# mlpc-ucsd/BDM

Measured on AMD Instinct MI355X. Metric: sampled shapes/sec (4096 pts, 1000 DDPM steps), higher is better.
Workload: dtype f32

## Files before the change

bdm_amd/csrc/sparse_conv_os.hip:

```cpp
#include <stdlib.h>

#include "../../include/bdm_hip.h"
#include "common.h"

using namespace bdm;

#include "sparse_h2_common.h"

#define OS_PAIRS 14

typedef __attribute__((ext_vector_type(4))) float f32x4a;
typedef float f32x4v_t __attribute__((ext_vector_type(4)));


#define TILE_REC 16
#define DILH_XCAP 1376

static void sconv_dil_geometry(int r, int half_tile, int *tile, int *xcap, int *tiles_max) {
  if (half_tile > 0) {
    *tile = half_tile;
    *xcap = DILH_XCAP;
  } else {
    *tile = r == 32 ? 512 : (r == 16 ? 256 : 128);
    *xcap = 3 * r * r;
// ... 222 lines not shown

extern "C" int bdm_voxel_dilate_slices(int r, int tile) {
  int tl, xcap, tiles_max;
  sconv_dil_geometry(r, half_tile_ok(r, tile) ? tile : 0, &tl, &xcap, &tiles_max);
  return tiles_max;
}

static int voxel_dilate_launch(int b, int r, int n_dil_max, const int *src, int thr, int *dil_list, int *dil_index, int *plane_start,
                               int *tile_start, int *class_count, int half_tile, void *stream) {
  BDM_REQUIRE(b >= 0 && (r == 8 || r == 16 || r == 32) && n_dil_max >= 1 && src && dil_list && dil_index && plane_start && tile_start,
              "voxel_dilate: bad arguments (r in {8, 16, 32})");
  BDM_REQUIRE(half_tile_ok(r, half_tile), "voxel_dilate: tile %d unsupported (0 = full tiles; 64 / 128 / 256: EXPERIMENTAL=1 builds)", half_tile);
  if (b == 0) return BDM_OK;
  int tile, xcap, tiles_max;
  sconv_dil_geometry(r, half_tile, &tile, &xcap, &tiles_max);
  BDM_REQUIRE(cdiv(r * r * r, tile) <= 1024, "voxel_dilate: more flat tiles than threads");
  const size_t smem = sizeof(unsigned) * (4 * (size_t)r * r + 1 + 32 + 2 * (r + 2));
  hipLaunchKernelGGL(vox_dilate_kernel, dim3(b), dim3(1024), smem, (hipStream_t)stream, r, n_dil_max, tile, xcap, tiles_max,
                     half_tile > 0 ? 1 : 0, src, thr, dil_list, dil_index, plane_start, tile_start, class_count);
  return launch_status("voxel_dilate");
}

extern "C" int bdm_voxel_dilate(int b, int r, int n_dil_max, const int *cnt, int *dil_list, int *dil_index, int *plane_start,
                                int *tile_start, int tile, void *stream) {
  return voxel_dilate_launch(b, r, n_dil_max, cnt, 0, dil_list, dil_index, plane_start, tile_start, nullptr, tile, stream);
}

extern "C" int bdm_voxel_dilate_again(int b, int r, int n_dil_max, const int *dil_index_in, int *dil_list, int *dil_index,
                                      int *plane_start, int *tile_start, int *class_count, int tile, void *stream) {
  BDM_REQUIRE(class_count != nullptr, "voxel_dilate_again: class_count is NULL");
  return voxel_dilate_launch(b, r, n_dil_max, dil_index_in, -1, dil_list, dil_index, plane_start, tile_start, class_count, tile, stream);
}

#ifdef DIL_TIMING
__device__ long long *g_dil_ts = nullptr;
extern "C" int bdm_debug_dil_timestamps(long long *buf) { return hipMemcpyToSymbol(HIP_SYMBOL(g_dil_ts), &buf, sizeof(buf)) == hipSuccess ? 0 : 1; }
#define DIL_STAMP(i) do { if (g_dil_ts && tid == 0) { g_dil_ts[(size_t)item * 8 + (i)] = wall_clock64();                                  \
    if ((i) == 0) g_dil_ts[(size_t)item * 8 + 7] = (long long)__builtin_amdgcn_s_getreg(63492) | ((long long)__builtin_amdgcn_s_getreg(63508) << 32); } } while (0)
#else
#define DIL_STAMP(i)
#endif

template <int MT, int NT, int NW, int R, bool H2IN>
__global__ __launch_bounds__(NW * 64) void sconv_dil_kernel(
    int C8, int Cout, int n_max, int n_dil_max, int xcap, const float4 *__restrict__ xr, const float *__restrict__ amax,
    const float4 *__restrict__ xconst, float x_inv_scale,
    const int *__restrict__ occ_index, const int *__restrict__ dil_list, const int *__restrict__ dil_index,
    const int *__restrict__ tile_start, const float4 *__restrict__ wq,
    const float *__restrict__ inv_scale, const float *__restrict__ bias, float *__restrict__ y, int compact, int gn_cg,
    double *__restrict__ gn_partial, int gn_slices, int nb_shapes, int ncb, int tiles_max, int *__restrict__ work_counter) {
  extern __shared__ __align__(16) float4 smem4[];
  constexpr int BM = 16 * MT, TILE = NT * NW * 16;
  constexpr int R2 = R * R, R3 = R2 * R;
  constexpr int NT_ = NW * 64;
  constexpr int WV = OS_PAIRS * 2 * 2 * BM, WI = (WV + NT_ - 1) / NT_;
  constexpr int NQ = OS_PAIRS / 2;
  constexpr int PF = MT * NT >= 16 ? 1 : 2;
  constexpr int NBLK = NT * NW, NB = MT * 4 * 2;
  float4 *Ws = smem4;
  float4 *Xs = smem4 + WV;
  const int XS = xcap + 128;
  __shared__ int s_item;
  __shared__ float s_osc[64], s_obi[64];

  const int tid0 = threadIdx.x;
  const int G = gn_partial != nullptr ? Cout / gn_cg : 0, S = gn_slices;
  const int items = tiles_max * ncb * nb_shapes;
  for (;;) {
    int tid = tid0;
    asm volatile("" : "+v"(tid));
    const int lane = tid & 63, wave = tid >> 6, l16 = lane & 15, kg = lane >> 4;
    __syncthreads();
    if (tid == 0) s_item = atomicAdd(work_counter, 1);
    __syncthreads();
    const int item = s_item;
    if (item >= items) break;
    const int bi = item % nb_shapes, m0 = ((item / nb_shapes) % ncb) * BM, tile = item / (nb_shapes * ncb);
  const int4 *te = reinterpret_cast<const int4 *>(tile_start + ((size_t)bi * tiles_max + tile) * TILE_REC);
  const int4 ta = te[0], tb = te[1];
  const int j0 = ta.x, jn = ta.y, v_first = ta.z, v_end = ta.w, k_lo = tb.x;
  const int tiles_live = tb.w, tile_x0 = tb.z >> 8, tile_x1 = tb.z & 255;
// ... 62 lines not shown
      *reinterpret_cast<f16x8 *>(&Xs[row]) = hi;
      *reinterpret_cast<f16x8 *>(&Xs[XS + row]) = lo;
    }
  };
  auto store_chunk = [&](int c8) {
#pragma unroll
    for (int u = 0; u < PF; ++u)
      if (tid + u * NT_ < nrows) {
        const float4 p = make_float4(xa[u][0][0], xa[u][0][1], xa[u][0][2], xa[u][0][3]);
        const float4 q = make_float4(xa[u][1][0], xa[u][1][1], xa[u][1][2], xa[u][1][3]);
        put(tid + u * NT_, p, q);
      }
    for (int row0 = tid + PF * NT_; row0 < nrows; row0 += 2 * NT_) {
      const int row1 = row0 + NT_, rc1 = min(row1, nrows - 1);
      float4 a0, a1, b0, b1;
      if (H2IN) {
        const float4 *src = xr + (((size_t)bi * C8 + c8) * 2) * n_max + k_lo;
        a0 = src[row0]; a1 = src[n_max + row0]; b0 = src[rc1]; b1 = src[n_max + rc1];
      } else {
        const float4 *src = xb + ((size_t)c8 * n_max + k_lo) * 2;
        a0 = src[2 * row0]; a1 = src[2 * row0 + 1]; b0 = src[2 * rc1]; b1 = src[2 * rc1 + 1];
      }
      put(row0, a0, a1);
      if (row1 < nrows) put(row1, b0, b1);
    }
    if (H2IN && tid < 128) *reinterpret_cast<f32x4v *>(&Xs[(tid >> 6) * XS + xcap + 64 + (tid & 63)]) = cr;
#pragma unroll
    for (int i = 0; i < WI; ++i) {
      const int e = tid + i * NT_;
      if (e < WV) *reinterpret_cast<f32x4v *>(&Ws[e]) = wr[i];
    }
  };

  if (!nothing) load_chunk(0);

  int rec[NT][NQ];
  unsigned amask = 0u;
  {
    const int pl0 = max(tile_x0 - 1, 0), pl1 = min(tile_x1 + 1, R - 1), n_oi = (pl1 - pl0 + 1) * R2;
    const bool staged = !nothing && n_oi * (int)sizeof(int) <= 2 * XS * (int)sizeof(float4);
    int *s_oi = reinterpret_cast<int *>(Xs);
    const int *oi = occ_index + (size_t)bi * R3;
    int vq[NT];
#pragma unroll
    for (int q = 0; q < NT; ++q) {
      const int j = j0 + (q * NW + wave) * 16 + l16;
      vq[q] = j < jn ? dl[j] : -1;
    }
    if (staged) {
      const int4 *src = reinterpret_cast<const int4 *>(oi + pl0 * R2);
      for (int e = tid; e < n_oi / 4; e += NT_) reinterpret_cast<int4 *>(s_oi)[e] = src[e];
      __syncthreads();
    }
#pragma unroll
    for (int q = 0; q < NT; ++q) {
      const int v = vq[q];
      const int vx = v / R2, vy = (v / R) % R, vz = v % R;
#pragma unroll
      for (int Q = 0; Q < NQ; ++Q) {
        const int t = 4 * Q + kg;
        int k = -1;
        bool inside = false;
        if (v >= 0 && t < 27) {
          const int gx = vx + t / 9 - 1, gy = vy + (t / 3) % 3 - 1, gz = vz + t % 3 - 1;
          inside = gx >= 0 && gx < R && gy >= 0 && gy < R && gz >= 0 && gz < R;
          if (inside) k = staged ? s_oi[((gx - pl0) * R + gy) * R + gz] : oi[(gx * R + gy) * R + gz];
        }
        const bool here = k >= k_lo && k - k_lo < nrows;
        const bool live = here || (H2IN && inside);
        if (__ballot(live) != 0ull) amask |= 1u << (Q * NT + q);
        rec[q][Q] = here ? k - k_lo : ((H2IN && inside) ? xcap + 64 + lane : xcap + lane);
      }
    }
    amask = __builtin_amdgcn_readfirstlane(amask);
  }
  DIL_STAMP(1);
  if (!nothing) {
    for (int c8 = 0; c8 < C8; ++c8) {
      __syncthreads();
      if (c8 == 0) DIL_STAMP(2);
      if (c8 == 0 && tid < 128) Xs[(tid >> 6) * XS + xcap + (tid & 63)] = make_float4(0.f, 0.f, 0.f, 0.f);
      store_chunk(c8);
      __syncthreads();
      if (c8 == 0) DIL_STAMP(3);
      if (c8 == 1) DIL_STAMP(4);
      if (c8 + 1 < C8) load_chunk(c8 + 1);
#pragma unroll
      for (int Q = 0; Q < NQ; ++Q) {
        const unsigned qm = (amask >> (Q * NT)) & ((1u << NT) - 1u);
        if (qm == 0u) continue;
        f16x8 fa[MT][2];
#pragma unroll
        for (int s = 0; s < 2; ++s)
#pragma unroll
          for (int mt = 0; mt < MT; ++mt) {
            const float4 t = wbase[Q * 8 * BM + s * 2 * BM + mt * 16];
            fa[mt][s] = *reinterpret_cast<const f16x8 *>(&t);
          }
#pragma unroll
        for (int q = 0; q < NT; ++q) {
          f16x8 fb[2];
#pragma unroll
          for (int s = 0; s < 2; ++s) {
            const float4 t = Xs[s * XS + rec[q][Q]];
            fb[s] = *reinterpret_cast<const f16x8 *>(&t);
          }
#pragma unroll
          for (int term = 0; term < 3; ++term)
#pragma unroll
            for (int mt = 0; mt < MT; ++mt)
              acc[mt][q] = __builtin_amdgcn_mfma_f32_16x16x32_f16(fa[mt][term == 0 ? 1 : 0], fb[term == 1 ? 1 : 0], acc[mt][q], 0, 0, 0);
        }
      }
    }
  }

  DIL_STAMP(5);
  __syncthreads();
  float *red = reinterpret_cast<float *>(smem4);
  float *otile = red + (NBLK + 1) * NB;
#pragma unroll
  for (int mt = 0; mt < MT; ++mt)
#pragma unroll
    for (int q = 0; q < NT; ++q) {
      const int jl = (q * NW + wave) * 16 + l16;
      const bool live = j0 + jl < jn;
      float bs = 0.f, bq = 0.f;
      f32x4a o = f32x4a{0.f, 0.f, 0.f, 0.f};
#pragma unroll
      for (int i = 0; i < 4; ++i) {
        const int m = m0 + mt * 16 + 4 * kg + i;
        if (m < Cout && live) {
          const float v = acc[mt][q][i] * s_osc[mt * 16 + 4 * kg + i] + s_obi[mt * 16 + 4 * kg + i];
          o[i] = v;
          bs += v;
          bq = __builtin_fmaf(v, v, bq);
        }
// ... 368 lines not shown
        float a = 0.f;
#pragma unroll
        for (int j = 0; j < NBLK; ++j) a += red[j * NB + e];
        red2[e] = a;
      }
      __syncthreads();
      const int ngt = BM / gn_cg;
      if (tid < ngt && m0 + tid * gn_cg < Cout) {
        double a = 0.0, qq = 0.0;
        const int nb4 = gn_cg / 4;
        for (int j = 0; j < nb4; ++j) {
          a += (double)red2[(tid * nb4 + j) * 2 + 0];
          qq += (double)red2[(tid * nb4 + j) * 2 + 1];
        }
        const double nfill = H2IN ? 0.0 : (double)((v_end - v_first) - (jn - j0));
        for (int c = 0; c < gn_cg; ++c) {
          const double bv = bias ? (double)bias[m0 + tid * gn_cg + c] : 0.0;
          a += nfill * bv;
          qq += nfill * bv * bv;
        }
        double *dst = gn_partial + (((size_t)bi * G + m0 / gn_cg + tid) * S + tile) * 2;
        dst[0] = a;
        dst[1] = qq;
      }
    }
    DIL_STAMP(6);
  }
}

#endif

static int sconv_dil_launch(bool h2in, int b, int cin, int cout, int r, int n_max, int n_dil_max, const void *xr, const float *amax,
                            const void *xconst, float x_inv_scale, const int *in_index, const int *dil_list, const int *dil_index,
                            const int *tile_start, const void *packed_w, const float *inv_scale, const float *bias, float *y,
                            int compact, int gn_cg, double *gn_partial, int *slices_out, int half_tile, int *work_counter,
                            void *stream) {
  BDM_REQUIRE(b >= 0 && cin >= 1 && cout >= 1 && n_max >= 1 && n_dil_max >= 1 && xr && (h2in ? xconst != nullptr : amax != nullptr) &&
                  in_index && dil_list && dil_index && tile_start && inv_scale && y && work_counter,
              "sparse_conv_dil: bad arguments");
  if (r != 8 && r != 16 && r != 32) {
    set_error("sparse_conv_dil: resolution %d unsupported (8, 16, 32)", r);
    return BDM_ERR_UNSUPPORTED;
  }
  BDM_REQUIRE(half_tile_ok(r, half_tile), "sparse_conv_dil: tile %d unsupported (0 = full tiles; 64 / 128 / 256: EXPERIMENTAL=1 builds)", half_tile);
  if (b == 0) return BDM_OK;
  const int c8 = (cin + 7) / 8;
  const int mi = cout > 32 ? 2 : 1;
  int tile, xcap, tiles;
  sconv_dil_geometry(r, half_tile, &tile, &xcap, &tiles);
  const int bm = 32 * mi, nblk = tile / 16, nb = (bm / 16) * 8, ncb = cdiv(cout, bm);
  size_t smem = half_tile ? 16 * (2 * ((size_t)xcap + 128))
                          : 16 * ((size_t)OS_PAIRS * 4 * bm + 2 * ((size_t)xcap + 128));
  const size_t smem_out = sizeof(float) * ((size_t)(nblk + 1) * nb + (compact ? 0 : (size_t)bm * tile));
  if (smem_out > smem) smem = smem_out;
  BDM_REQUIRE(!half_tile || smem + 1024 <= 81920, "sparse_conv_dil: the half-tile form needs two workgroups per CU (%zu bytes of LDS)", smem);
  static int cus[16] = {0};
  int dev = 0;
  (void)hipGetDevice(&dev);
  if (dev < 0 || dev >= 16 || cus[dev] == 0) {
    hipDeviceProp_t prop;
    const int n = hipGetDeviceProperties(&prop, dev) == hipSuccess ? prop.multiProcessorCount : 256;
    if (dev >= 0 && dev < 16) cus[dev] = n > 0 ? n : 256;
  }
  const int ncu = ((dev >= 0 && dev < 16) ? cus[dev] : 256) * (half_tile ? 2 : 1);
  const long long items = (long long)tiles * ncb * b;
  dim3 grid((unsigned)(items < ncu ? items : ncu));
  hipStream_t s = (hipStream_t)stream;
  const int slices = h2in ? tiles + 27 : tiles;
  if (gn_partial != nullptr) {
    BDM_REQUIRE(gn_cg >= 4 && (gn_cg & (gn_cg - 1)) == 0 && bm % gn_cg == 0 && cout % gn_cg == 0,
                "sparse_conv_dil: GroupNorm statistics need a power-of-two channels-per-group dividing %d (got cg=%d)", bm, gn_cg);
    if (slices_out) *slices_out = slices;
  }
#define DIL_LAUNCH_(MT, NT, NW, R, H)                                                                                      \
  do {                                                                                                                     \
    BDM_ALLOW_LDS((sconv_dil_kernel<MT, NT, NW, R, H>), smem);                                                             \
    hipLaunchKernelGGL((sconv_dil_kernel<MT, NT, NW, R, H>), grid, dim3(NW * 64), smem, s, c8, cout, n_max, n_dil_max,     \
                       xcap, (const float4 *)xr, amax, (const float4 *)xconst, x_inv_scale, in_index, dil_list, dil_index, \
                       tile_start, (const float4 *)packed_w, inv_scale, bias, y, compact, gn_cg, gn_partial, slices, b,    \
                       ncb, tiles, work_counter);                                                                          \
  } while (0)
#define DIL_LAUNCH(MT, NT, NW, R) do { if (h2in) DIL_LAUNCH_(MT, NT, NW, R, true); else DIL_LAUNCH_(MT, NT, NW, R, false); } while (0)
#define DILH_LAUNCH_(MT, NT, R, H)                                                                                         \
  do {                                                                                                                     \
    BDM_ALLOW_LDS((sconv_dilh_kernel<MT, NT, R, H>), smem);                                                                \
    hipLaunchKernelGGL((sconv_dilh_kernel<MT, NT, R, H>), grid, dim3(256), smem, s, c8, cout, n_max, n_dil_max,            \
                       (const float4 *)xr, amax, (const float4 *)xconst, x_inv_scale, in_index, dil_list, dil_index,       \
                       tile_start, (const float4 *)packed_w, inv_scale, bias, y, compact, gn_cg, gn_partial, slices, b,    \
                       ncb, tiles, work_counter);                                                                          \
  } while (0)
#define DILH_LAUNCH(MT, NT, R) do { if (h2in) DILH_LAUNCH_(MT, NT, R, true); else DILH_LAUNCH_(MT, NT, R, false); } while (0)
#define DILH_PICK(NT, R) do { if (mi == 2) DILH_LAUNCH(4, NT, R); else DILH_LAUNCH(2, NT, R); } while (0)
#ifdef BDM_EXPERIMENTAL
  if (half_tile) {
    const int nt = half_tile / 64;
    if (r == 32) { if (nt == 4) DILH_PICK(4, 32); else if (nt == 2) DILH_PICK(2, 32); else DILH_PICK(1, 32); }
    else if (r == 16) { if (nt == 4) DILH_PICK(4, 16); else if (nt == 2) DILH_PICK(2, 16); else DILH_PICK(1, 16); }
    else { if (nt == 2) DILH_PICK(2, 8); else DILH_PICK(1, 8); }
    return launch_status("sparse_conv_dil (half tiles)");
  }
#endif
  if (r == 32) { if (mi == 2) DIL_LAUNCH(4, 4, 8, 32); else DIL_LAUNCH(2, 4, 8, 32); }
  else if (r == 16) { if (mi == 2) DIL_LAUNCH(4, 2, 8, 16); else DIL_LAUNCH(2, 2, 8, 16); }
  else { if (mi == 2) DIL_LAUNCH(4, 1, 8, 8); else DIL_LAUNCH(2, 1, 8, 8); }
#undef DIL_LAUNCH
#undef DIL_LAUNCH_
#undef DILH_PICK
#undef DILH_LAUNCH
#undef DILH_LAUNCH_
  return launch_status("sparse_conv_dil");
}

extern "C" int bdm_sparse_conv_dil(int b, int cin, int cout, int r, int n_max, int n_dil_max, const void *xr, const float *amax,
                                   const int *occ_index, const int *dil_list, const int *dil_index, const int *tile_start,
                                   const void *packed_w, const float *inv_scale, const float *bias, float *y,
                                   int compact, int tile, int *work_counter, void *stream) {
  return sconv_dil_launch(false, b, cin, cout, r, n_max, n_dil_max, xr, amax, nullptr, 0.f, occ_index, dil_list, dil_index, tile_start,
                          packed_w, inv_scale, bias, y, compact, 0, nullptr, nullptr, tile, work_counter, stream);
}

extern "C" int bdm_sparse_conv_dil_gn(int b, int cin, int cout, int r, int n_max, int n_dil_max, const void *xr, const float *amax,
                                      const int *occ_index, const int *dil_list, const int *dil_index, const int *tile_start,
                                      const void *packed_w, const float *inv_scale, const float *bias,
                                      float *y, int compact, int groups, void *gn_partial, int *slices_out, int tile,
                                      int *work_counter, void *stream) {
  BDM_REQUIRE(groups >= 1 && cout % groups == 0 && gn_partial != nullptr && slices_out != nullptr, "sparse_conv_dil_gn: bad arguments");
  return sconv_dil_launch(false, b, cin, cout, r, n_max, n_dil_max, xr, amax, nullptr, 0.f, occ_index, dil_list, dil_index, tile_start,
                          packed_w, inv_scale, bias, y, compact, cout / groups, (double *)gn_partial, slices_out, tile, work_counter, stream);
}

extern "C" int bdm_sparse_conv_dil_h2_gn(int b, int cin, int cout, int r, int n_rows_max, int n_dil_max, const void *rows_h2,
                                         const void *xconst, float x_inv_scale, const int *in_index, const int *dil_list,
                                         const int *dil_index, const int *tile_start, const void *packed_w, const float *inv_scale,
                                         const float *bias, float *y, int groups, void *gn_partial, int *slices_out, int tile,
                                         int *work_counter, void *stream) {
  BDM_REQUIRE(groups >= 1 && cout % groups == 0 && gn_partial != nullptr && slices_out != nullptr && x_inv_scale > 0.f,
              "sparse_conv_dil_h2_gn: bad arguments");
  return sconv_dil_launch(true, b, cin, cout, r, n_rows_max, n_dil_max, rows_h2, nullptr, xconst, x_inv_scale, in_index, dil_list,
                          dil_index, tile_start, packed_w, inv_scale, bias, y, 1, cout / groups, (double *)gn_partial, slices_out, tile,
                          work_counter, stream);
}
```

bdm_amd/ops.py:

```python
import ctypes
import os

import torch

from . import _lib as L
from . import tape


def _bcl(t):
    if t.dtype != torch.float32:
        raise L.BdmHipError(f"expected float32, got {t.dtype}")
    B, C = t.shape[0], t.shape[1]
    if B * C > 0 and t.is_contiguous():
        l = t.numel() // (B * C)
        return t, B, C, l, C * l, l
    l = 1
    for s in t.shape[2:]:
        l *= s
    dense, exp = True, 1
    for d in range(t.dim() - 1, 1, -1):
        if t.shape[d] != 1 and t.stride(d) != exp:
            dense = False
        exp *= t.shape[d]
    if dense and C > 1 and t.stride(1) < l:
# ... 794 lines not shown
_amax_rings = {}
_static_epoch = 0
_static_epochs = 0


class static_step:

    def __enter__(self):
        global _static_epoch, _static_epochs
        _static_epochs += 1
        _static_epoch = _static_epochs

    def __exit__(self, *exc):
        global _static_epoch
        _static_epoch = 0
        return False


def _amax_slot(device):
    dev = torch.device(device)
    key = (str(device), torch._C._cuda_getCurrentRawStream(dev.index if dev.index is not None else torch._C._cuda_getDevice()))
    ring = _amax_rings.get(key)
    if ring is None or ring[1] >= ring[0].shape[0] or ring[2] != _static_epoch:
        ring = [torch.zeros(256, dtype=torch.float32, device=device), 0, _static_epoch]
        _amax_rings[key] = ring
    slot = ring[0][ring[1]:ring[1] + 1]
    ring[1] += 1
    return slot


class VoxelPlan:
    __slots__ = ("r", "n", "n_max", "coords", "norm_coords", "vox_coords", "ind", "cnt", "ws", "occ_index", "occ_list", "n_occ", "rowocc",
                 "ready", "stream", "dil_list", "dil_index", "plane_start", "tile_start", "n_dil_max",
                 "d2_list", "d2_index", "d2_tiles", "d2_class_count", "tile", "d2_tile")

    def __init__(self, vox_coords, r, norm_coords=None, coords=None):
        B, _, n = vox_coords.shape
        dev, r3 = vox_coords.device, r ** 3
        self.ready = self.stream = None
        self.r, self.n, self.n_max = int(r), n, min(n, r3)
        self.coords, self.norm_coords, self.vox_coords = coords, norm_coords, vox_coords
        self.ind = torch.empty(B, n, dtype=torch.int32, device=dev)
        self.cnt = torch.empty(B, r3, dtype=torch.int32, device=dev)
        self.ws = torch.empty(L.lib().bdm_voxelize_workspace_bytes(B, n, r), dtype=torch.uint8, device=dev)
        self.occ_index = torch.empty(B, r3, dtype=torch.int32, device=dev)
        self.occ_list = torch.empty(B, self.n_max, dtype=torch.int32, device=dev)
        self.n_occ = torch.empty(B, dtype=torch.int32, device=dev)
        self.rowocc = torch.empty(B, r * r, dtype=torch.uint8, device=dev)
        self.dil_list = self.d2_list = None


_plan_cache = {}


def clear_plan_cache():
    _plan_cache.clear()


def voxel_plan(coords, r, eps=0.0, dilate=False):
    key = (coords.data_ptr(), coords._version, tuple(coords.shape), int(r))
    p = _plan_cache.get(key)
    if p is not None:
        ready = getattr(p, "ready", None)
        if ready is not None:
            if torch.cuda.current_stream(coords.device) != getattr(p, "stream", None):
                tape.wait_event(ready)
                p.ready = None
        return p
    lib = L.lib()
    B, _, n = coords.shape
    norm_coords, vox_coords = voxel_coords(coords, r, eps)
    p = VoxelPlan(vox_coords, r, norm_coords, coords)
    L.check(lib.bdm_voxelize_plan_full(B, n, r, p.n_max, L.ptr(p.vox_coords), L.ptr(p.ind), L.ptr(p.cnt), L.ptr(p.ws),
                                       L.ptr(p.occ_index), L.ptr(p.occ_list), L.ptr(p.n_occ), L.ptr(p.rowocc), L.stream()),
            "voxelize_plan_full")
    if dilate:
        plan_dilation(p)
        if dilate == 2:
            plan_dilation2(p)
    p.stream = torch.cuda.current_stream(coords.device) if coords.is_cuda else None
    _plan_cache[key] = p
    return p
# ... 6 lines not shown
TILE_REC = 16
DIL_TILE = os.environ.get("BDM_DIL_TILE", "0")


def dil_tile(batch, n_points, r, second):
    if r not in (8, 16, 32) or DIL_TILE in ("0", "", "auto"):
        return 0
    if not L.has_experimental():
        raise L.BdmHipError(f"BDM_DIL_TILE={DIL_TILE}: the half-tile list convolution belongs to the experimental kernel families; "
                            "rebuild with `make -C bdm_amd/csrc EXPERIMENTAL=1`")
    return min(int(DIL_TILE), 128) if r == 8 else int(DIL_TILE)


DILATED_PLAN = True


def plan_dilation(p):
    if getattr(p, "dil_list", None) is not None:
        return p
    p.dil_list = p.dil_index = p.plane_start = p.tile_start = None
    p.n_dil_max = 0
    if not DILATED_PLAN or p.r not in (8, 16, 32):
        return p
    lib, B, r = L.lib(), p.cnt.shape[0], p.r
    dev = p.cnt.device
    p.n_dil_max = r ** 3
    p.tile = dil_tile(B, p.n, r, second=False)
    p.dil_list = torch.empty(B, p.n_dil_max, dtype=torch.int32, device=dev)
    p.dil_index = torch.empty(B, r ** 3, dtype=torch.int32, device=dev)
    p.plane_start = torch.empty(B, r + 2, dtype=torch.int32, device=dev)
    p.tile_start = torch.empty(B, lib.bdm_voxel_dilate_slices(r, p.tile), TILE_REC, dtype=torch.int32, device=dev)
    L.check(lib.bdm_voxel_dilate(B, r, p.n_dil_max, L.ptr(p.cnt), L.ptr(p.dil_list), L.ptr(p.dil_index), L.ptr(p.plane_start),
                                 L.ptr(p.tile_start), p.tile, L.stream()), "voxel_dilate")
    return p


def plan_dilation2(p):
    if getattr(p, "d2_list", None) is not None:
        return p
    plan_dilation(p)
    p.d2_list = p.d2_index = p.d2_tiles = p.d2_class_count = None
    if p.dil_list is None:
        return p
    lib, B, r = L.lib(), p.cnt.shape[0], p.r
    dev = p.cnt.device
    p.d2_tile = dil_tile(B, p.n, r, second=True)
    p.d2_list = torch.empty(B, p.n_dil_max, dtype=torch.int32, device=dev)
    p.d2_index = torch.empty(B, r ** 3, dtype=torch.int32, device=dev)
    ps = torch.empty(B, r + 2, dtype=torch.int32, device=dev)
    p.d2_tiles = torch.empty(B, lib.bdm_voxel_dilate_slices(r, p.d2_tile), TILE_REC, dtype=torch.int32, device=dev)
    p.d2_class_count = torch.empty(B, 27, dtype=torch.int32, device=dev)
    L.check(lib.bdm_voxel_dilate_again(B, r, p.n_dil_max, L.ptr(p.dil_index), L.ptr(p.d2_list), L.ptr(p.d2_index), L.ptr(ps),
                                       L.ptr(p.d2_tiles), L.ptr(p.d2_class_count), p.d2_tile, L.stream()), "voxel_dilate_again")
    return p


HOIST_CONDITIONING = os.environ.get("BDM_HOIST", "1") == "1"


def three_nn_search(points_coords, centers_coords):
    pc, cc = points_coords.contiguous(), centers_coords.contiguous()
    B, _, n = pc.shape
    m = cc.shape[2]
    idx = torch.empty(B, 3, n, dtype=torch.int32, device=pc.device)
    w = torch.empty(B, 3, n, dtype=torch.float32, device=pc.device)
    L.check(L.lib().bdm_three_nn_search(B, m, n, L.ptr(pc), L.ptr(cc), L.ptr(idx), L.ptr(w), L.stream()), "three_nn_search")
    return idx, w


def _fill_conditioning_map(feat, wf, out):
    xt = wf.t().contiguous()[None]
    for b in range(feat.shape[0]):
        pointwise_conv(xt, feat[b], out=out[b:b + 1])


def refresh_conditioning_maps(feat, maps):
    for key, ent in list(maps.items()):
        if len(ent) != 4:
            continue
        if ent[0] != ent[2]._version:
            del maps[key]
        else:
            _fill_conditioning_map(feat, ent[3]().contiguous(), ent[1])


class Conditioning:
# ... 198 lines not shown
class CompactGrid:

    def __init__(self, rows, plan, bias, channels):
        self.rows, self.plan, self.bias, self.channels = rows, plan, bias, channels

    is_cuda = property(lambda self: self.rows.is_cuda)
    device = property(lambda self: self.rows.device)

    def dense(self):
        B, r3, C = self.rows.shape[0], self.plan.r ** 3, self.channels
        out = self.bias.detach().view(1, C, 1).expand(B, C, r3).contiguous()
        idx = self.plan.dil_index.long()
        for b in range(B):
            v = torch.nonzero(idx[b] >= 0).squeeze(1)
            out[b, :, v] = self.rows[b, idx[b, v]].t()
        return out


def sparse_first_conv_os(features, plan, packed, bias, cout, gn_groups=None, compact=False):
    plan_dilation(plan)
    if plan.dil_list is None:
        raise L.BdmHipError(f"sparse_first_conv_os: resolution {plan.r} has no dilated plan (8, 16, 32)")
    f, B, C, n, bs_f, ld_f = _bcl(features)
    dev, lib, r = f.device, L.lib(), plan.r
    packed_w, inv_scale = packed
    xr, slots = _records_f32((f, B, C, n, bs_f, ld_f), plan, extra=1)
    amax, counter = slots[:B], slots[B:]
    if compact:
        y = torch.empty(B, plan.n_dil_max, cout, dtype=torch.float32, device=dev)
        out = CompactGrid(y, plan, bias, cout)
    else:
        y = out = torch.empty(B, cout, r ** 3, dtype=torch.float32, device=dev)
    args = (B, C, cout, r, plan.n_max, plan.n_dil_max, L.ptr(xr), L.ptr(amax), L.ptr(plan.occ_index), L.ptr(plan.dil_list),
            L.ptr(plan.dil_index), L.ptr(plan.tile_start), L.ptr(packed_w), L.ptr(inv_scale), L.ptr(bias), L.ptr(y), 1 if compact else 0)
    if gn_groups:
        tiles = plan.tile_start.shape[1]
        partial = torch.empty(B, gn_groups, tiles, 2, dtype=torch.float64, device=dev)
        slices = ctypes.c_int(0)
        L.check(lib.bdm_sparse_conv_dil_gn(*args, int(gn_groups), L.ptr(partial), ctypes.byref(slices), plan.tile, L.ptr(counter), L.stream()),
                "sparse_conv_dil_gn")
        return out, (partial, tiles, int(gn_groups))
    L.check(lib.bdm_sparse_conv_dil(*args, plan.tile, L.ptr(counter), L.stream()), "sparse_conv_dil")
    return out


def to_h2_rows(x, plan, gn, stats, swish=True, saturated=None, bias=None):
    plan_dilation(plan)
    lib = L.lib()
    compact = isinstance(x, CompactGrid)
    src = x.rows if compact else x.contiguous()
    bias = x.bias if compact else bias
    B, C, V = src.shape[0], (x.channels if compact else src.shape[1]), plan.r ** 3
    dev = src.device
    s = float(h2_activation_scale(gn))
    C8 = (C + 7) // 8
    rows = torch.empty(B, C8, 2, plan.n_dil_max, 8, dtype=torch.float16, device=dev)
    const_h2 = torch.empty(B, C8, 2, 8, dtype=torch.float16, device=dev)
    const_f32 = torch.empty(B, C, dtype=torch.float32, device=dev)
    partial, slices, groups = stats
    L.check(lib.bdm_group_norm_to_h2_rows(B, C, V, groups, L.ptr(src), 0 if compact else 1, plan.n_dil_max, L.ptr(plan.dil_list),
                                          L.ptr(plan.tile_start), plan.tile_start.shape[1], L.ptr(bias), L.ptr(gn.weight), L.ptr(gn.bias),
                                          L.c_float(gn.eps), 1 if swish else 0, L.c_float(s), L.ptr(rows), L.ptr(const_h2), L.ptr(const_f32),
                                          L.ptr(partial), slices, L.ptr(saturated), L.stream()), "group_norm_to_h2_rows")
    return rows, const_h2, const_f32, 1.0 / s


def conv_class_pack(weight):
    cout, cin = weight.shape[:2]
    lib = L.lib()
    wsum = torch.empty(lib.bdm_conv3d_class_weight_elems(cout, cin), dtype=torch.float64, device=weight.device)
    L.check(lib.bdm_conv3d_class_weight_sums(cout, cin, L.ptr(weight.contiguous()), L.ptr(wsum), L.stream()), "conv3d_class_weight_sums")
    return wsum


def second_conv_rows(rows_h2, const_h2, const_f32, x_inv_scale, plan, packed, wsum, bias, cin, cout, groups=8):
    plan_dilation2(plan)
    lib, B, r = L.lib(), rows_h2.shape[0], plan.r
    dev = rows_h2.device
    packed_w, inv_scale = packed
    y = torch.empty(B, plan.n_dil_max, cout, dtype=torch.float32, device=dev)
    tiles = plan.d2_tiles.shape[1]
    partial = torch.empty(B, groups, tiles + 27, 2, dtype=torch.float64, device=dev)
    counter = amax_slots(dev, 1)
    slices = ctypes.c_int(0)
    L.check(lib.bdm_sparse_conv_dil_h2_gn(B, cin, cout, r, plan.n_dil_max, plan.n_dil_max, L.ptr(rows_h2), L.ptr(const_h2), L.c_float(x_inv_scale),
                                          L.ptr(plan.dil_index), L.ptr(plan.d2_list), L.ptr(plan.d2_index), L.ptr(plan.d2_tiles), L.ptr(packed_w),
                                          L.ptr(inv_scale), L.ptr(bias), L.ptr(y), int(groups), L.ptr(partial), ctypes.byref(slices), plan.d2_tile,
                                          L.ptr(counter), L.stream()), "sparse_conv_dil_h2_gn")
    assert slices.value == tiles + 27
    class_vals = torch.empty(B, 27, cout, dtype=torch.float32, device=dev)
    L.check(lib.bdm_conv3d_class_constants(B, cin, cout, L.ptr(wsum), L.ptr(bias), L.ptr(const_f32), L.ptr(plan.d2_class_count), L.ptr(class_vals),
                                           int(groups), L.ptr(partial), tiles + 27, tiles, L.stream()), "conv3d_class_constants")
    return y, class_vals, (partial, tiles + 27)


def se_gate_gn_rows(rows, class_vals, plan, stats, gn, w1, w2, pf=None, n_points=0):
    partial, slices = stats
    B, C = rows.shape[0], rows.shape[2]
    dev, lib = rows.device, L.lib()
    V = plan.r ** 3
    mean = torch.empty(B, C, dtype=torch.float32, device=dev)
    coef = torch.empty(B, C, 2, dtype=torch.float32, device=dev)
    gate = torch.empty(B, C, dtype=torch.float32, device=dev)
    part = torch.empty(lib.bdm_se_gate_gn_rows_workspace_elems(B, C), dtype=torch.float32, device=dev)
    args = (B, C, w1.shape[0], V, gn.num_groups, L.ptr(rows), plan.n_dil_max, L.ptr(plan.d2_tiles), plan.d2_tiles.shape[1], L.ptr(class_vals),
            L.ptr(plan.d2_class_count), L.ptr(partial), slices, L.ptr(gn.weight), L.ptr(gn.bias), L.c_float(gn.eps), L.ptr(w1), L.ptr(w2), L.ptr(part),
            L.ptr(mean), L.ptr(coef), L.ptr(gate))
    if pf is not None:
        (pp, ps, pg), pgn = pf
        pf_coef = torch.empty(B, C, 2, dtype=torch.float32, device=dev)
        L.check(lib.bdm_se_gate_gn_rows_pf(*args, L.ptr(pp), ps, pg, int(n_points), L.ptr(pgn.weight), L.ptr(pgn.bias), L.c_float(pgn.eps),
                                           L.ptr(pf_coef), L.stream()), "se_gate_gn_rows_pf")
        return gate, coef, pf_coef
    L.check(lib.bdm_se_gate_gn_rows(*args, L.stream()), "se_gate_gn_rows")
    return gate, coef


def devoxelize_gn_gate_add_rows(norm_coords, rows, class_vals, plan, coef, gate=None, add=None, add_coef=None):
    B, C = rows.shape[0], rows.shape[2]
# ... 72 lines not shown
```

include/bdm_hip.h:

```cpp
#ifndef BDM_HIP_H
#define BDM_HIP_H

#include <stddef.h>
#include <stdint.h>

#ifdef __cplusplus
extern "C" {
#endif

const char *bdm_last_error(void);
int bdm_abi_version(void);


int bdm_furthest_point_sampling(int b, int n, int m, const float *coords, int *indices,
                                float *centers_out, void *stream);

int bdm_gather_features_forward(int b, int c, int n, int m, const float *features,
                                const int *indices, float *out, void *stream);

int bdm_ball_query(int b, int n, int m, float radius, int u, const float *centers,
                   const float *points, int *neighbors, void *stream);

int bdm_grouping_forward(int b, int c, int n, int m, int u, const float *features,
                         const int *indices, float *out, void *stream);
// ... 215 lines not shown
                              int ld_f, const int *cnt, const void *plan_workspace, const int *occ_list,
                              const int *n_occ, float *xc, void *stream);
int bdm_sparse_conv_pack_weights(int cout, int cin, const float *w, float *wt, void *stream);
int bdm_sparse_conv_gemm(int b, int n_max, int cin, int n27, const float *xc, const float *wt,
                         const int *n_occ, float *y, void *stream);
int bdm_sparse_conv_gather(int b, int cout, int r, int n_max, const float *y, const int *occ_index,
                           const unsigned char *rowocc, const float *bias, float *out, void *stream);
int bdm_sparse_conv_gather_gn(int b, int cout, int r, int n_max, const float *y, const int *occ_index,
                              const unsigned char *rowocc, const float *bias, float *out, int groups, void *gn_partial,
                              void *stream);

int bdm_sparse_voxel_features_f32(int b, int c, int n, int r, int n_max, const float *features, long long bs_f,
                                  int ld_f, const int *cnt, const void *plan_workspace, const int *occ_list,
                                  const int *n_occ, void *xr, float *amax, void *stream);
#ifdef BDM_EXPERIMENTAL
size_t bdm_sparse_conv_fused_weight_elems(int cout, int cin);
int bdm_sparse_conv_fused_pack_weights(int cout, int cin, const float *w, void *packed, float *scale_ws,
                                       float *inv_scale, void *stream);
int bdm_sparse_conv_fused(int b, int cin, int cout, int r, int n_max, const void *xr, const float *amax,
                          const void *packed_w, const float *inv_scale, const int *occ_list, const int *n_occ,
                          const float *bias, float *out, void *stream);
#endif

size_t bdm_sparse_conv_h2_weight_elems(int cout, int cin);
int bdm_sparse_conv_pack_weights_h2(int cout, int cin, const float *w, void *packed, float *scale_ws,
                                    float *inv_scale, void *stream);
int bdm_sparse_split_h2(int b, int cin, int n_max, const void *xr, const float *amax, void *xh, void *stream);
int bdm_sparse_conv_gemm_h2(int b, int n_max, int cin, int cout, const void *xh, const float *amax, const void *packed_w,
                            const float *inv_scale, const int *n_occ, float *y, void *stream);
int bdm_sparse_conv_gemm_h2_cb(int b, int n_max, int cin, int cout, const void *xh, const float *amax, const void *packed_w,
                               const float *inv_scale, const int *n_occ, const float *col_bias, long long bs_cb, float *y, void *stream);

int bdm_voxel_dilate_slices(int r, int tile);
int bdm_voxel_dilate(int b, int r, int n_dil_max, const int *cnt, int *dil_list, int *dil_index, int *plane_start, int *tile_start,
                     int tile, void *stream);
int bdm_sparse_conv_dil(int b, int cin, int cout, int r, int n_max, int n_dil_max, const void *xr, const float *amax,
                        const int *occ_index, const int *dil_list, const int *dil_index, const int *tile_start,
                        const void *packed_w, const float *inv_scale, const float *bias, float *y, int compact, int tile,
                        int *work_counter, void *stream);
int bdm_sparse_conv_dil_gn(int b, int cin, int cout, int r, int n_max, int n_dil_max, const void *xr, const float *amax,
                           const int *occ_index, const int *dil_list, const int *dil_index, const int *tile_start,
                           const void *packed_w, const float *inv_scale, const float *bias, float *y, int compact, int groups,
                           void *gn_partial, int *slices_out, int tile, int *work_counter, void *stream);

int bdm_voxel_dilate_again(int b, int r, int n_dil_max, const int *dil_index_in, int *dil_list, int *dil_index, int *plane_start,
                           int *tile_start, int *class_count, int tile, void *stream);
int bdm_group_norm_to_h2_rows(int b, int c, int v, int groups, const float *x, int dense_in, int n_rows_max, const int *dil_list,
                              const int *tile_start, int tiles_max, const float *bias, const float *gamma, const float *beta,
                              float eps, int act, float act_scale, void *rows_h2, void *const_h2, float *const_f32,
                              const void *partial, int slices, unsigned int *saturated, void *stream);
int bdm_sparse_conv_dil_h2_gn(int b, int cin, int cout, int r, int n_rows_max, int n_dil_max, const void *rows_h2, const void *xconst,
                              float x_inv_scale, const int *in_index, const int *dil_list, const int *dil_index,
                              const int *tile_start, const void *packed_w, const float *inv_scale, const float *bias, float *y,
                              int groups, void *gn_partial, int *slices_out, int tile, int *work_counter, void *stream);
size_t bdm_conv3d_class_weight_elems(int cout, int cin);
int bdm_conv3d_class_weight_sums(int cout, int cin, const float *w, void *wsum, void *stream);
int bdm_conv3d_class_constants(int b, int cin, int cout, const void *wsum, const float *bias, const float *const_f32,
                               const int *class_count, float *class_vals, int groups, void *gn_partial, int slices, int slice0,
                               void *stream);
size_t bdm_se_gate_gn_rows_workspace_elems(int b, int c);
int bdm_se_gate_gn_rows(int b, int c, int hidden, int v, int groups, const float *rows, int n_rows_max, const int *tile_start,
                        int tiles_max, const float *class_vals, const int *class_count, const void *gn_partial, int slices,
                        const float *gamma, const float *beta, float eps, const float *w1, const float *w2, float *part_ws,
                        float *mean_ws, float *coef, float *gate, void *stream);
int bdm_se_gate_gn_rows_pf(int b, int c, int hidden, int v, int groups, const float *rows, int n_rows_max, const int *tile_start,
                           int tiles_max, const float *class_vals, const int *class_count, const void *gn_partial, int slices,
                           const float *gamma, const float *beta, float eps, const float *w1, const float *w2, float *part_ws,
                           float *mean_ws, float *coef, float *gate, const void *pf_partial, int pf_slices, int pf_groups, int pf_n,
                           const float *pf_gamma, const float *pf_beta, float pf_eps, float *pf_coef, void *stream);
int bdm_devoxelize_gn_gate_add_rows(int b, int c, int n, int r, const float *coords, const float *rows, int n_rows_max,
                                    const int *dil_index, const float *class_vals, const float *coef, const float *gate,
                                    const float *add, long long bs_a, int ld_a, float *out, long long bs_o, int ld_o, void *stream);
int bdm_devoxelize_gn_gate_add_rows_pf(int b, int c, int n, int r, const float *coords, const float *rows, int n_rows_max,
                                       const int *dil_index, const float *class_vals, const float *coef, const float *gate,
                                       const float *add, long long bs_a, int ld_a, const float *add_coef, float *out, long long bs_o,
                                       int ld_o, void *stream);


int bdm_ddpm_step(long long n, const float *x, const float *eps, const float *noise,
                  float sqrt_beta_prod, float sqrt_alpha_prod, float coef_x0, float coef_x,
                  float sigma, float *out, void *stream);
int bdm_ddpm_step_dev(long long n, const float *x, const float *eps, const float *noise, const float *coef,
                      float *out, void *stream);

int bdm_ddim_step(long long n, const float *x, const float *eps, const float *noise, float sqrt_beta_prod,
                  float sqrt_alpha_prod, float coef_x0, float coef_eps, float sigma, float *out, void *stream);

// ... 90 lines not shown
```

Before: 2.953.

## Precompute dilated-conv neighbour records and masks once per voxel plan

```diff
diff --git a/bdm_amd/csrc/sparse_conv_os.hip b/bdm_amd/csrc/sparse_conv_os.hip
--- a/bdm_amd/csrc/sparse_conv_os.hip
+++ b/bdm_amd/csrc/sparse_conv_os.hip
@@ -278,6 +278,77 @@
   return voxel_dilate_launch(b, r, n_dil_max, dil_index_in, -1, dil_list, dil_index, plane_start, tile_start, class_count, tile, stream);
 }
 
+template <int R>
+__global__ __launch_bounds__(256) void dil_records_kernel(int n_dil_max, int nblk, int tiles_max, int xcap, int const_form,
+                                                          const int *__restrict__ in_index, const int *__restrict__ dil_list,
+                                                          const int *__restrict__ tile_start, uint4 *__restrict__ records,
+                                                          unsigned *__restrict__ masks) {
+  constexpr int R2 = R * R, R3 = R2 * R, NQ = OS_PAIRS / 2, NW = 8;
+  const int tid = threadIdx.x, lane = tid & 63, l16 = lane & 15, kg = lane >> 4;
+  const int g = blockIdx.x * 4 + (tid >> 6), tile = g / nblk, nb = g - tile * nblk, bi = blockIdx.y;
+  if (tile >= tiles_max) return;
+  const int4 *te = reinterpret_cast<const int4 *>(tile_start + ((size_t)bi * tiles_max + tile) * TILE_REC);
+  const int4 ta = te[0], tb = te[1];
+  const int j0 = ta.x, jn = ta.y, k_lo = tb.x, nrows = jn <= j0 ? 0 : tb.y;
+  if (tile >= max(tb.w, 1)) return;
+  const int NT = nblk / NW, q = nb / NW;
+  const int j = j0 + nb * 16 + l16;
+  const int v = j < jn ? dil_list[(size_t)bi * n_dil_max + j] : -1;
+  const int vx = v / R2, vy = (v / R) % R, vz = v % R;
+  const int *oi = in_index + (size_t)bi * R3;
+  int k[NQ];
+  bool inside[NQ];
+#pragma unroll
+  for (int Q = 0; Q < NQ; ++Q) {
+    const int t = 4 * Q + kg;
+    k[Q] = -1;
+    inside[Q] = false;
+    if (v >= 0 && t < 27) {
+      const int gx = vx + t / 9 - 1, gy = vy + (t / 3) % 3 - 1, gz = vz + t % 3 - 1;
+      inside[Q] = gx >= 0 && gx < R && gy >= 0 && gy < R && gz >= 0 && gz < R;
+      if (inside[Q]) k[Q] = oi[(gx * R + gy) * R + gz];
+    }
+  }
+  unsigned h[8], m = 0u;
+  h[7] = (unsigned)(xcap + lane) << 4;
+#pragma unroll
+  for (int Q = 0; Q < NQ; ++Q) {
+    const bool here = k[Q] >= k_lo && k[Q] - k_lo < nrows;
+    const bool cst = const_form && inside[Q];
+    if (__ballot(here || cst) != 0ull) m |= 1u << (Q * NT + q);
+    h[Q] = (unsigned)(here ? k[Q] - k_lo : (cst ? xcap + 64 + lane : xcap + lane)) << 4;
+  }
+  if (j < jn) records[((size_t)bi * n_dil_max + j) * 4 + kg] = make_uint4(h[0] | (h[1] << 16), h[2] | (h[3] << 16), h[4] | (h[5] << 16), h[6] | (h[7] << 16));
+  if (lane == 0) masks[((size_t)bi * tiles_max + tile) * nblk + nb] = m;
+}
+
+extern "C" size_t bdm_voxel_dilate_records_elems(int b, int n_dil_max) { return b > 0 && n_dil_max > 0 ? (size_t)b * (size_t)n_dil_max * 16 : 0; }
+
+extern "C" size_t bdm_voxel_dilate_masks_elems(int b, int r) {
+  int tile, xcap, tiles_max;
+  sconv_dil_geometry(r, 0, &tile, &xcap, &tiles_max);
+  return b > 0 ? (size_t)b * tiles_max * (tile / 16) : 0;
+}
+
+extern "C" int bdm_voxel_dilate_records(int b, int r, int n_dil_max, const int *in_index, const int *dil_list, const int *tile_start,
+                                        int const_form, void *records, void *masks, void *stream) {
+  BDM_REQUIRE(b >= 0 && (r == 8 || r == 16 || r == 32) && n_dil_max >= 1 && in_index && dil_list && tile_start && records && masks,
+              "voxel_dilate_records: bad arguments (r in {8, 16, 32})");
+  if (b == 0) return BDM_OK;
+  int tile, xcap, tiles_max;
+  sconv_dil_geometry(r, 0, &tile, &xcap, &tiles_max);
+  BDM_REQUIRE((xcap + 128) * 16 <= 65536, "voxel_dilate_records: %d input rows do not fit a 16-bit byte offset", xcap);
+  const int nblk = tile / 16;
+  const dim3 grid((unsigned)(tiles_max * nblk / 4), (unsigned)b);
+  hipStream_t s = (hipStream_t)stream;
+#define REC_LAUNCH(R)                                                                                                   \
+  hipLaunchKernelGGL((dil_records_kernel<R>), grid, dim3(256), 0, s, n_dil_max, nblk, tiles_max, xcap, const_form ? 1 : 0, \
+                     in_index, dil_list, tile_start, (uint4 *)records, (unsigned *)masks)
+  if (r == 32) REC_LAUNCH(32); else if (r == 16) REC_LAUNCH(16); else REC_LAUNCH(8);
+#undef REC_LAUNCH
+  return launch_status("voxel_dilate_records");
+}
+
 #ifdef DIL_TIMING
 __device__ long long *g_dil_ts = nullptr;
 extern "C" int bdm_debug_dil_timestamps(long long *buf) { return hipMemcpyToSymbol(HIP_SYMBOL(g_dil_ts), &buf, sizeof(buf)) == hipSuccess ? 0 : 1; }
@@ -292,7 +363,8 @@
     int C8, int Cout, int n_max, int n_dil_max, int xcap, const float4 *__restrict__ xr, const float *__restrict__ amax,
     const float4 *__restrict__ xconst, float x_inv_scale,
     const int *__restrict__ occ_index, const int *__restrict__ dil_list, const int *__restrict__ dil_index,
-    const int *__restrict__ tile_start, const float4 *__restrict__ wq,
+    const int *__restrict__ tile_start, const uint4 *__restrict__ rec_tab, const unsigned *__restrict__ mask_tab,
+    const float4 *__restrict__ wq,
     const float *__restrict__ inv_scale, const float *__restrict__ bias, float *__restrict__ y, int compact, int gn_cg,
     double *__restrict__ gn_partial, int gn_slices, int nb_shapes, int ncb, int tiles_max, int *__restrict__ work_counter) {
   extern __shared__ __align__(16) float4 smem4[];
@@ -421,11 +493,22 @@
     }
   };
 
+  unsigned rec[NT][4];
+  unsigned amask = 0u;
+  if (rec_tab != nullptr) {
+#pragma unroll
+    for (int q = 0; q < NT; ++q) {
+      const int j = j0 + (q * NW + wave) * 16 + l16;
+      const unsigned z = (unsigned)((xcap + lane) << 4) * 0x10001u;
+      const uint4 t = j < jn ? rec_tab[((size_t)bi * n_dil_max + j) * 4 + kg] : make_uint4(z, z, z, z);
+      rec[q][0] = t.x; rec[q][1] = t.y; rec[q][2] = t.z; rec[q][3] = t.w;
+      amask |= mask_tab[((size_t)bi * tiles_max + tile) * (NT * NW) + q * NW + wave];
+    }
+  }
   if (!nothing) load_chunk(0);
-
-  int rec[NT][NQ];
-  unsigned amask = 0u;
-  {
+  if (rec_tab != nullptr) {
+    amask = __builtin_amdgcn_readfirstlane(amask);
+  } else {
     const int pl0 = max(tile_x0 - 1, 0), pl1 = min(tile_x1 + 1, R - 1), n_oi = (pl1 - pl0 + 1) * R2;
     const bool staged = !nothing && n_oi * (int)sizeof(int) <= 2 * XS * (int)sizeof(float4);
     int *s_oi = reinterpret_cast<int *>(Xs);
@@ -458,8 +541,10 @@
         const bool here = k >= k_lo && k - k_lo < nrows;
         const bool live = here || (H2IN && inside);
         if (__ballot(live) != 0ull) amask |= 1u << (Q * NT + q);
-        rec[q][Q] = here ? k - k_lo : ((H2IN && inside) ? xcap + 64 + lane : xcap + lane);
-      }
+        const unsigned o = (unsigned)(here ? k - k_lo : ((H2IN && inside) ? xcap + 64 + lane : xcap + lane)) << 4;
+        if ((Q & 1) == 0) rec[q][Q >> 1] = o; else rec[q][Q >> 1] |= o << 16;
+      }
+      rec[q][3] |= (unsigned)((xcap + lane) << 4) << 16;
     }
     amask = __builtin_amdgcn_readfirstlane(amask);
   }
@@ -475,6 +560,10 @@
       if (c8 == 1) DIL_STAMP(4);
       if (c8 + 1 < C8) load_chunk(c8 + 1);
 #pragma unroll
+      for (int q = 0; q < NT; ++q)
+#pragma unroll
+        for (int w = 0; w < 4; ++w) asm volatile("" : "+v"(rec[q][w]));
+#pragma unroll
       for (int Q = 0; Q < NQ; ++Q) {
         const unsigned qm = (amask >> (Q * NT)) & ((1u << NT) - 1u);
         if (qm == 0u) continue;
@@ -491,7 +580,8 @@
           f16x8 fb[2];
 #pragma unroll
           for (int s = 0; s < 2; ++s) {
-            const float4 t = Xs[s * XS + rec[q][Q]];
+            const unsigned o = (rec[q][Q >> 1] >> (16 * (Q & 1))) & 0xffffu;
+            const float4 t = *reinterpret_cast<const float4 *>(reinterpret_cast<const char *>(Xs + s * XS) + o);
             fb[s] = *reinterpret_cast<const f16x8 *>(&t);
           }
 #pragma unroll
@@ -926,9 +1016,9 @@
 
 static int sconv_dil_launch(bool h2in, int b, int cin, int cout, int r, int n_max, int n_dil_max, const void *xr, const float *amax,
                             const void *xconst, float x_inv_scale, const int *in_index, const int *dil_list, const int *dil_index,
-                            const int *tile_start, const void *packed_w, const float *inv_scale, const float *bias, float *y,
-                            int compact, int gn_cg, double *gn_partial, int *slices_out, int half_tile, int *work_counter,
-                            void *stream) {
+                            const int *tile_start, const void *records, const void *masks, const void *packed_w,
+                            const float *inv_scale, const float *bias, float *y, int compact, int gn_cg, double *gn_partial,
+                            int *slices_out, int half_tile, int *work_counter, void *stream) {
   BDM_REQUIRE(b >= 0 && cin >= 1 && cout >= 1 && n_max >= 1 && n_dil_max >= 1 && xr && (h2in ? xconst != nullptr : amax != nullptr) &&
                   in_index && dil_list && dil_index && tile_start && inv_scale && y && work_counter,
               "sparse_conv_dil: bad arguments");
@@ -937,6 +1027,8 @@
     return BDM_ERR_UNSUPPORTED;
   }
   BDM_REQUIRE(half_tile_ok(r, half_tile), "sparse_conv_dil: tile %d unsupported (0 = full tiles; 64 / 128 / 256: EXPERIMENTAL=1 builds)", half_tile);
+  BDM_REQUIRE((records == nullptr) == (masks == nullptr) && (records == nullptr || half_tile == 0),
+              "sparse_conv_dil: the plan's neighbour records come with their masks, for full tiles only");
   if (b == 0) return BDM_OK;
   const int c8 = (cin + 7) / 8;
   const int mi = cout > 32 ? 2 : 1;
@@ -971,8 +1063,8 @@
     BDM_ALLOW_LDS((sconv_dil_kernel<MT, NT, NW, R, H>), smem);                                                             \
     hipLaunchKernelGGL((sconv_dil_kernel<MT, NT, NW, R, H>), grid, dim3(NW * 64), smem, s, c8, cout, n_max, n_dil_max,     \
                        xcap, (const float4 *)xr, amax, (const float4 *)xconst, x_inv_scale, in_index, dil_list, dil_index, \
-                       tile_start, (const float4 *)packed_w, inv_scale, bias, y, compact, gn_cg, gn_partial, slices, b,    \
-                       ncb, tiles, work_counter);                                                                          \
+                       tile_start, (const uint4 *)records, (const unsigned *)masks, (const float4 *)packed_w, inv_scale,   \
+                       bias, y, compact, gn_cg, gn_partial, slices, b, ncb, tiles, work_counter);                          \
   } while (0)
 #define DIL_LAUNCH(MT, NT, NW, R) do { if (h2in) DIL_LAUNCH_(MT, NT, NW, R, true); else DIL_LAUNCH_(MT, NT, NW, R, false); } while (0)
 #define DILH_LAUNCH_(MT, NT, R, H)                                                                                         \
@@ -1007,30 +1099,30 @@
 
 extern "C" int bdm_sparse_conv_dil(int b, int cin, int cout, int r, int n_max, int n_dil_max, const void *xr, const float *amax,
                                    const int *occ_index, const int *dil_list, const int *dil_index, const int *tile_start,
-                                   const void *packed_w, const float *inv_scale, const float *bias, float *y,
-                                   int compact, int tile, int *work_counter, void *stream) {
+                                   const void *records, const void *masks, const void *packed_w, const float *inv_scale,
+                                   const float *bias, float *y, int compact, int tile, int *work_counter, void *stream) {
   return sconv_dil_launch(false, b, cin, cout, r, n_max, n_dil_max, xr, amax, nullptr, 0.f, occ_index, dil_list, dil_index, tile_start,
-                          packed_w, inv_scale, bias, y, compact, 0, nullptr, nullptr, tile, work_counter, stream);
+                          records, masks, packed_w, inv_scale, bias, y, compact, 0, nullptr, nullptr, tile, work_counter, stream);
 }
 
 extern "C" int bdm_sparse_conv_dil_gn(int b, int cin, int cout, int r, int n_max, int n_dil_max, const void *xr, const float *amax,
                                       const int *occ_index, const int *dil_list, const int *dil_index, const int *tile_start,
-                                      const void *packed_w, const float *inv_scale, const float *bias,
-                                      float *y, int compact, int groups, void *gn_partial, int *slices_out, int tile,
+                                      const void *records, const void *masks, const void *packed_w, const float *inv_scale,
+                                      const float *bias, float *y, int compact, int groups, void *gn_partial, int *slices_out, int tile,
                                       int *work_counter, void *stream) {
   BDM_REQUIRE(groups >= 1 && cout % groups == 0 && gn_partial != nullptr && slices_out != nullptr, "sparse_conv_dil_gn: bad arguments");
   return sconv_dil_launch(false, b, cin, cout, r, n_max, n_dil_max, xr, amax, nullptr, 0.f, occ_index, dil_list, dil_index, tile_start,
-                          packed_w, inv_scale, bias, y, compact, cout / groups, (double *)gn_partial, slices_out, tile, work_counter, stream);
+                          records, masks, packed_w, inv_scale, bias, y, compact, cout / groups, (double *)gn_partial, slices_out, tile, work_counter, stream);
 }
 
 extern "C" int bdm_sparse_conv_dil_h2_gn(int b, int cin, int cout, int r, int n_rows_max, int n_dil_max, const void *rows_h2,
                                          const void *xconst, float x_inv_scale, const int *in_index, const int *dil_list,
-                                         const int *dil_index, const int *tile_start, const void *packed_w, const float *inv_scale,
-                                         const float *bias, float *y, int groups, void *gn_partial, int *slices_out, int tile,
+                                         const int *dil_index, const int *tile_start, const void *records, const void *masks,
+                                         const void *packed_w, const float *inv_scale, const float *bias, float *y, int groups, void *gn_partial, int *slices_out, int tile,
                                          int *work_counter, void *stream) {
   BDM_REQUIRE(groups >= 1 && cout % groups == 0 && gn_partial != nullptr && slices_out != nullptr && x_inv_scale > 0.f,
               "sparse_conv_dil_h2_gn: bad arguments");
   return sconv_dil_launch(true, b, cin, cout, r, n_rows_max, n_dil_max, rows_h2, nullptr, xconst, x_inv_scale, in_index, dil_list,
-                          dil_index, tile_start, packed_w, inv_scale, bias, y, 1, cout / groups, (double *)gn_partial, slices_out, tile,
+                          dil_index, tile_start, records, masks, packed_w, inv_scale, bias, y, 1, cout / groups, (double *)gn_partial, slices_out, tile,
                           work_counter, stream);
 }
diff --git a/bdm_amd/ops.py b/bdm_amd/ops.py
--- a/bdm_amd/ops.py
+++ b/bdm_amd/ops.py
@@ -850,7 +850,8 @@
 class VoxelPlan:
     __slots__ = ("r", "n", "n_max", "coords", "norm_coords", "vox_coords", "ind", "cnt", "ws", "occ_index", "occ_list", "n_occ", "rowocc",
                  "ready", "stream", "dil_list", "dil_index", "plane_start", "tile_start", "n_dil_max",
-                 "d2_list", "d2_index", "d2_tiles", "d2_class_count", "tile", "d2_tile")
+                 "d2_list", "d2_index", "d2_tiles", "d2_class_count", "tile", "d2_tile",
+                 "records", "masks", "d2_records", "d2_masks")
 
     def __init__(self, vox_coords, r, norm_coords=None, coords=None):
         B, _, n = vox_coords.shape
@@ -866,6 +867,7 @@
         self.n_occ = torch.empty(B, dtype=torch.int32, device=dev)
         self.rowocc = torch.empty(B, r * r, dtype=torch.uint8, device=dev)
         self.dil_list = self.d2_list = None
+        self.records = self.masks = self.d2_records = self.d2_masks = None
 
 
 _plan_cache = {}
@@ -938,7 +940,22 @@
     p.tile_start = torch.empty(B, lib.bdm_voxel_dilate_slices(r, p.tile), TILE_REC, dtype=torch.int32, device=dev)
     L.check(lib.bdm_voxel_dilate(B, r, p.n_dil_max, L.ptr(p.cnt), L.ptr(p.dil_list), L.ptr(p.dil_index), L.ptr(p.plane_start),
                                  L.ptr(p.tile_start), p.tile, L.stream()), "voxel_dilate")
+    p.records, p.masks = _dil_records(p, p.occ_index, p.dil_list, p.tile_start, p.tile, const_form=False)
     return p
+
+
+DIL_RECORDS = os.environ.get("BDM_DIL_RECORDS", "1") != "0"
+
+
+def _dil_records(p, in_index, dil_list, tile_start, tile, const_form):
+    if tile != 0 or not DIL_RECORDS:
+        return None, None
+    lib, B, dev = L.lib(), in_index.shape[0], in_index.device
+    records = torch.empty(lib.bdm_voxel_dilate_records_elems(B, p.n_dil_max), dtype=torch.int32, device=dev)
+    masks = torch.empty(lib.bdm_voxel_dilate_masks_elems(B, p.r), dtype=torch.int32, device=dev)
+    L.check(lib.bdm_voxel_dilate_records(B, p.r, p.n_dil_max, L.ptr(in_index), L.ptr(dil_list), L.ptr(tile_start), 1 if const_form else 0,
+                                         L.ptr(records), L.ptr(masks), L.stream()), "voxel_dilate_records")
+    return records, masks
 
 
 def plan_dilation2(p):
@@ -958,6 +975,7 @@
     p.d2_class_count = torch.empty(B, 27, dtype=torch.int32, device=dev)
     L.check(lib.bdm_voxel_dilate_again(B, r, p.n_dil_max, L.ptr(p.dil_index), L.ptr(p.d2_list), L.ptr(p.d2_index), L.ptr(ps),
                                        L.ptr(p.d2_tiles), L.ptr(p.d2_class_count), p.d2_tile, L.stream()), "voxel_dilate_again")
+    p.d2_records, p.d2_masks = _dil_records(p, p.dil_index, p.d2_list, p.d2_tiles, p.d2_tile, const_form=True)
     return p
 
 
@@ -1222,7 +1240,8 @@
     else:
         y = out = torch.empty(B, cout, r ** 3, dtype=torch.float32, device=dev)
     args = (B, C, cout, r, plan.n_max, plan.n_dil_max, L.ptr(xr), L.ptr(amax), L.ptr(plan.occ_index), L.ptr(plan.dil_list),
-            L.ptr(plan.dil_index), L.ptr(plan.tile_start), L.ptr(packed_w), L.ptr(inv_scale), L.ptr(bias), L.ptr(y), 1 if compact else 0)
+            L.ptr(plan.dil_index), L.ptr(plan.tile_start), L.ptr(plan.records), L.ptr(plan.masks), L.ptr(packed_w), L.ptr(inv_scale), L.ptr(bias),
+            L.ptr(y), 1 if compact else 0)
     if gn_groups:
         tiles = plan.tile_start.shape[1]
         partial = torch.empty(B, gn_groups, tiles, 2, dtype=torch.float64, device=dev)
@@ -1274,7 +1293,8 @@
     counter = amax_slots(dev, 1)
     slices = ctypes.c_int(0)
     L.check(lib.bdm_sparse_conv_dil_h2_gn(B, cin, cout, r, plan.n_dil_max, plan.n_dil_max, L.ptr(rows_h2), L.ptr(const_h2), L.c_float(x_inv_scale),
-                                          L.ptr(plan.dil_index), L.ptr(plan.d2_list), L.ptr(plan.d2_index), L.ptr(plan.d2_tiles), L.ptr(packed_w),
+                                          L.ptr(plan.dil_index), L.ptr(plan.d2_list), L.ptr(plan.d2_index), L.ptr(plan.d2_tiles), L.ptr(plan.d2_records),
+                                          L.ptr(plan.d2_masks), L.ptr(packed_w),
                                           L.ptr(inv_scale), L.ptr(bias), L.ptr(y), int(groups), L.ptr(partial), ctypes.byref(slices), plan.d2_tile,
                                           L.ptr(counter), L.stream()), "sparse_conv_dil_h2_gn")
     assert slices.value == tiles + 27
diff --git a/include/bdm_hip.h b/include/bdm_hip.h
--- a/include/bdm_hip.h
+++ b/include/bdm_hip.h
@@ -271,15 +271,20 @@
                                const float *inv_scale, const int *n_occ, const float *col_bias, long long bs_cb, float *y, void *stream);
 
 int bdm_voxel_dilate_slices(int r, int tile);
+size_t bdm_voxel_dilate_records_elems(int b, int n_dil_max);
+size_t bdm_voxel_dilate_masks_elems(int b, int r);
+int bdm_voxel_dilate_records(int b, int r, int n_dil_max, const int *in_index, const int *dil_list, const int *tile_start,
+                             int const_form, void *records, void *masks, void *stream);
 int bdm_voxel_dilate(int b, int r, int n_dil_max, const int *cnt, int *dil_list, int *dil_index, int *plane_start, int *tile_start,
                      int tile, void *stream);
 int bdm_sparse_conv_dil(int b, int cin, int cout, int r, int n_max, int n_dil_max, const void *xr, const float *amax,
                         const int *occ_index, const int *dil_list, const int *dil_index, const int *tile_start,
-                        const void *packed_w, const float *inv_scale, const float *bias, float *y, int compact, int tile,
-                        int *work_counter, void *stream);
+                        const void *records, const void *masks, const void *packed_w, const float *inv_scale, const float *bias,
+                        float *y, int compact, int tile, int *work_counter, void *stream);
 int bdm_sparse_conv_dil_gn(int b, int cin, int cout, int r, int n_max, int n_dil_max, const void *xr, const float *amax,
                            const int *occ_index, const int *dil_list, const int *dil_index, const int *tile_start,
-                           const void *packed_w, const float *inv_scale, const float *bias, float *y, int compact, int groups,
+                           const void *records, const void *masks, const void *packed_w, const float *inv_scale,
+                           const float *bias, float *y, int compact, int groups,
                            void *gn_partial, int *slices_out, int tile, int *work_counter, void *stream);
 
 int bdm_voxel_dilate_again(int b, int r, int n_dil_max, const int *dil_index_in, int *dil_list, int *dil_index, int *plane_start,
@@ -290,8 +295,9 @@
                               const void *partial, int slices, unsigned int *saturated, void *stream);
 int bdm_sparse_conv_dil_h2_gn(int b, int cin, int cout, int r, int n_rows_max, int n_dil_max, const void *rows_h2, const void *xconst,
                               float x_inv_scale, const int *in_index, const int *dil_list, const int *dil_index,
-                              const int *tile_start, const void *packed_w, const float *inv_scale, const float *bias, float *y,
-                              int groups, void *gn_partial, int *slices_out, int tile, int *work_counter, void *stream);
+                              const int *tile_start, const void *records, const void *masks, const void *packed_w,
+                              const float *inv_scale, const float *bias, float *y, int groups, void *gn_partial, int *slices_out,
+                              int tile, int *work_counter, void *stream);
 size_t bdm_conv3d_class_weight_elems(int cout, int cin);
 int bdm_conv3d_class_weight_sums(int cout, int cin, const float *w, void *wsum, void *stream);
 int bdm_conv3d_class_constants(int b, int cin, int cout, const void *wsum, const float *bias, const float *const_f32,
```

Result: no change. 2.963, median of 6 (+0.3%).
